# obeychoi0120/wseg

Hardware: AMD Instinct MI355X
Metric: training images/sec at B=16x448x448 (contrast_train step) (higher is better)
Workload: dtype bf16; 1 GPU; ResNet-38 contrast, synthetic VOC 448x448, B=16/GPU, procedural weights, dropout on, fused HIP loss; global_batch=16, parallelism=dp1, seed=0

## Files before the change

wseg_amd/csrc/conv_igemm.hip:

```cpp
#include <stdlib.h>
#include <algorithm>
#include "common.h"
#include "conv_wgrad_kernels.h"
#include "conv_probes.h"

namespace {

constexpr int BN = 128, ROWB = 128;
constexpr int B_TILE = BN * ROWB;
constexpr int EPI_LD = BN + 4;

struct Args {
  wseg_conv_desc d;
  int M;
  int taps;
  int cpt;
  int cpt2;
  int krow;
  int ntn;
  int nwg;
  int row0;
  int perm;
  int Q1, Q2;
};

struct PermRow { wseg_rowgeo g; int cls; long true_row; };
__device__ __forceinline__ PermRow perm_decode(const Args& a, int m) {
  const wseg_conv_desc& d = a.d;
  PermRow r;
  int rr = m, H = d.OH, W = d.OW, Q = a.Q1, seg = 0;
  if (d.OH2 != 0 && rr >= 4 * a.Q1) { rr -= 4 * a.Q1; H = d.OH2; W = d.OW2; Q = a.Q2; seg = 1; }
  const int cls = rr / Q, rem = rr - cls * Q;
  const int hw2 = (H >> 1) * (W >> 1), w2 = W >> 1;
  const int n = rem / hw2, rem2 = rem - n * hw2;
  const int i = rem2 / w2, j = rem2 - i * w2;
  r.g.oy = 2 * i + (cls >> 1); r.g.ox = 2 * j + (cls & 1);
  r.g.n_glob = seg ? d.N + n : n;
  r.g.IH = seg ? d.IH2 : d.IH; r.g.IW = seg ? d.IW2 : d.IW;
  r.g.in_base = seg ? (long)d.N * d.IH * d.IW + (long)n * d.IH2 * d.IW2 : (long)n * d.IH * d.IW;
  r.cls = seg * 4 + cls;
  r.true_row = seg ? (long)d.N * d.OH * d.OW + ((long)n * H + r.g.oy) * W + r.g.ox : ((long)n * H + r.g.oy) * W + r.g.ox;
  return r;
}

__device__ __forceinline__ float elu1(float x) { return x > 0.f ? x : expm1f(x); }

__device__ __forceinline__ void epilogue_coeffs(const wseg_conv_desc& d, int n0, int cv, float (&sc)[8], float (&sh)[8]) {
  const int oc_raw = n0 + cv;
  const int oc = oc_raw < d.OC ? oc_raw : 0;
#pragma unroll
  for (int e = 0; e < 8; ++e) { sc[e] = 1.f; sh[e] = 0.f; }
  if (d.scale != nullptr) load8<WSEG_F32>(d.scale, oc, sc);
  if (d.shift != nullptr) load8<WSEG_F32>(d.shift, oc, sh);
}

template <int DT, int EPI, int ROWS>
__device__ __forceinline__ void epilogue_image(const wseg_conv_desc& d, int M, const float* img, int m0, int n0, int tid,
                                               const float (&sc)[8], const float (&sh)[8]) {
  constexpr int NT = 256, GPR = BN / 8;
  constexpr int RPS = NT / GPR;
  constexpr int SWEEPS = ROWS / RPS;
  constexpr int CHK = SWEEPS < 4 ? SWEEPS : 4;
  static_assert(NT % GPR == 0 && ROWS % RPS == 0 && SWEEPS % CHK == 0, "epilogue geometry");
  const int cv = (tid % GPR) * 8;
  const int oc_raw = n0 + cv;
  const bool col_ok = oc_raw < d.OC;
  const int oc = col_ok ? oc_raw : 0;
  const bool has_pre = d.r_pre != nullptr, has_post = d.r_post != nullptr, has_mask = d.mask != nullptr;
  const bool has_drop = d.drop != nullptr;
#pragma unroll 1
  for (int c0 = 0; c0 < SWEEPS; c0 += CHK) {
    float rpre[CHK][8], rpost[CHK][8], mk[CHK][8], dr[CHK][8];
    size_t mrow[CHK];
    bool ok[CHK];
#pragma unroll
    for (int j = 0; j < CHK; ++j) {
      const int row = ((c0 + j) * NT + tid) / GPR;
      ok[j] = col_ok && (m0 + row) < M;
      mrow[j] = ok[j] ? (size_t)(m0 + row) : 0;
    }
    if (has_pre) {
#pragma unroll
      for (int j = 0; j < CHK; ++j) load8<DT>(d.r_pre, mrow[j] * d.ld_rpre + oc, rpre[j]);
    }
    if (has_post) {
#pragma unroll
      for (int j = 0; j < CHK; ++j) load8<DT>(d.r_post, mrow[j] * d.ld_rpost + oc, rpost[j]);
    }
    if (EPI == 1 && has_mask) {
#pragma unroll
      for (int j = 0; j < CHK; ++j) load8<DT>(d.mask, mrow[j] * d.ld_mask + oc, mk[j]);
    }
    if (EPI < 2 && has_drop) {
#pragma unroll
      for (int j = 0; j < CHK; ++j) load8<WSEG_F32>(d.drop, (size_t)wseg_decode_row(d, (int)mrow[j]).n_glob * d.OC + oc, dr[j]);
    }
#pragma unroll
    for (int j = 0; j < CHK; ++j) {
      const int row = ((c0 + j) * NT + tid) / GPR;
      const size_t m = mrow[j];
      float v[8];
      const f32x4 p0 = *reinterpret_cast<const f32x4*>(&img[row * EPI_LD + cv]);
      const f32x4 p1 = *reinterpret_cast<const f32x4*>(&img[row * EPI_LD + cv + 4]);
#pragma unroll
      for (int e = 0; e < 4; ++e) { v[e] = p0[e]; v[4 + e] = p1[e]; }
      if (has_pre) {
#pragma unroll
        for (int e = 0; e < 8; ++e) v[e] += rpre[j][e];
      }
      if constexpr (EPI == 0) {
        if (has_post) {
#pragma unroll
          for (int e = 0; e < 8; ++e) v[e] += rpost[j][e];
        }
        if (d.relu_lt > 0) {
#pragma unroll
          for (int e = 0; e < 8; ++e) if (oc + e < d.relu_lt) v[e] = fmaxf(v[e], 0.f);
        }
        if (d.out != nullptr && ok[j]) store8<DT>(d.out, m * d.ld_out + oc, v);
        if (d.out2 != nullptr) {
          float t[8];
#pragma unroll
          for (int e = 0; e < 8; ++e) {
            float x = v[e] * sc[e] + sh[e];
            if (d.relu_out2) x = fmaxf(x, 0.f);
            if (has_drop) x *= dr[j][e];
            t[e] = x;
          }
          if (ok[j]) store8<DT>(d.out2, m * d.ld_out2 + oc, t);
        }
      } else if constexpr (EPI == 1) {
        float o[8];
#pragma unroll
        for (int e = 0; e < 8; ++e) {
          float x = v[e] * sc[e];
          if (has_drop) x *= dr[j][e];
          if (has_mask) x = mk[j][e] > 0.f ? x : 0.f;
          if (has_post) x += rpost[j][e];
          o[e] = x;
        }
        if (ok[j]) store8<DT>(d.out, m * d.ld_out + oc, o);
      } else if constexpr (EPI == 2) {
#pragma unroll
        for (int e = 0; e < 8; ++e) v[e] = fmaxf(v[e], 0.f);
        if (ok[j]) store8<DT>(d.out, m * d.ld_out + oc, v);
      } else {
#pragma unroll
        for (int e = 0; e < 8; ++e) v[e] = elu1(v[e]);
        if (ok[j]) store8<DT>(d.out, m * d.ld_out + oc, v);
      }
    }
  }
}

template <int DT> struct raw8;
template <> struct raw8<WSEG_BF16> {
  uint4 q;
  __device__ __forceinline__ void load(const void* p, size_t i) { q = *reinterpret_cast<const uint4*>((const bf16_t*)p + i); }
  __device__ __forceinline__ void unpack(float (&v)[8]) const {
    const unsigned w[4] = {q.x, q.y, q.z, q.w};
#pragma unroll
    for (int j = 0; j < 4; ++j) { v[2 * j] = __uint_as_float(w[j] << 16); v[2 * j + 1] = __uint_as_float(w[j] & 0xFFFF0000u); }
  }
};
template <> struct raw8<WSEG_F32X3> {
  f32x4 q0, q1;
  __device__ __forceinline__ void load(const void* p, size_t i) {
    q0 = *reinterpret_cast<const f32x4*>((const float*)p + i); q1 = *reinterpret_cast<const f32x4*>((const float*)p + i + 4);
  }
  __device__ __forceinline__ void unpack(float (&v)[8]) const {
#pragma unroll
    for (int e = 0; e < 4; ++e) { v[e] = q0[e]; v[4 + e] = q1[e]; }
  }
};

template <int EPI, int NI, int I0, int NB, int DT>
__device__ __forceinline__ void wave_local_epilogue_batch(const Args& a, float* wimg, int lane, int mw0, int oc, bool col_ok,
                                                          const float (&sc)[8], const float (&sh)[8], const f32x4 (&acc)[NI][4]) {
  constexpr int WLD = 64 + 4;
  const wseg_conv_desc& d = a.d;
  const int frow = lane & 15, fk = lane >> 4;
  const int vr = lane >> 3, vg = lane & 7;
  const bool ld_ok_ = WSEG_DIAG_EPI_LOADS();
  const bool has_pre = d.r_pre != nullptr && ld_ok_, has_post = d.r_post != nullptr && ld_ok_, has_mask = EPI == 1 && d.mask != nullptr && ld_ok_;
  const bool has_drop = EPI < 2 && d.drop != nullptr && ld_ok_;
  const bool res_is_pre = has_pre;
  const bool post_in_step = has_pre && has_post;
  const void* res_p = res_is_pre ? d.r_pre : d.r_post;
  const size_t res_ld = res_is_pre ? d.ld_rpre : d.ld_rpost;
  const bool has_res = has_pre || has_post;
  int mrow[NB][2]; bool ok[NB][2];
  raw8<DT> qres[NB][2], qmk[NB][2];
#pragma unroll
  for (int i = 0; i < NB; ++i)
#pragma unroll
    for (int t = 0; t < 2; ++t) {
      const int m = mw0 + (I0 + i) * 16 + vr + 8 * t;
      ok[i][t] = col_ok && m < a.M;
      mrow[i][t] = ok[i][t] ? (a.perm ? (int)perm_decode(a, m).true_row : m) : 0;
      ok[i][t] = ok[i][t] && WSEG_DIAG_EPI_STORES();
      if (has_res) qres[i][t].load(res_p, (size_t)mrow[i][t] * res_ld + oc);
      if (has_mask) qmk[i][t].load(d.mask, (size_t)mrow[i][t] * d.ld_mask + oc);
    }
#pragma unroll
  for (int i = 0; i < NB; ++i) {
    float rpost[2][8], dr[2][8];
    if (post_in_step) {
#pragma unroll
      for (int t = 0; t < 2; ++t) load8<DT>(d.r_post, (size_t)mrow[i][t] * d.ld_rpost + oc, rpost[t]);
    }
    if (has_drop) {
#pragma unroll
      for (int t = 0; t < 2; ++t) load8<WSEG_F32>(d.drop, (size_t)wseg_decode_row(d, mrow[i][t]).n_glob * d.OC + oc, dr[t]);
    }
#pragma unroll
    for (int j = 0; j < 4; ++j)
#pragma unroll
      for (int e = 0; e < 4; ++e) wimg[(fk * 4 + e) * WLD + j * 16 + frow] = acc[I0 + i][j][e];
    asm volatile("s_waitcnt lgkmcnt(0)" ::: "memory");
#pragma unroll
    for (int t = 0; t < 2; ++t) {
      float v[8];
      {
        const f32x4 p0 = *reinterpret_cast<const f32x4*>(&wimg[(vr + 8 * t) * WLD + vg * 8]);
        const f32x4 p1 = *reinterpret_cast<const f32x4*>(&wimg[(vr + 8 * t) * WLD + vg * 8 + 4]);
#pragma unroll
        for (int e = 0; e < 4; ++e) { v[e] = p0[e]; v[4 + e] = p1[e]; }
      }
      const size_t m = (size_t)mrow[i][t];
      float res[8];
      if (has_res) qres[i][t].unpack(res);
      if (has_pre) {
#pragma unroll
        for (int e = 0; e < 8; ++e) v[e] += res[e];
      }
      if (!post_in_step && has_post) {
#pragma unroll
        for (int e = 0; e < 8; ++e) rpost[t][e] = res[e];
      }
      if constexpr (EPI == 0) {
        if (has_post) {
#pragma unroll
          for (int e = 0; e < 8; ++e) v[e] += rpost[t][e];
        }
        if (d.relu_lt > 0) {
#pragma unroll
          for (int e = 0; e < 8; ++e) if (oc + e < d.relu_lt) v[e] = fmaxf(v[e], 0.f);
        }
        if (d.out != nullptr && ok[i][t]) store8<DT>(d.out, m * d.ld_out + oc, v);
        if (d.out2 != nullptr) {
          float o2[8];
#pragma unroll
          for (int e = 0; e < 8; ++e) {
            float x = v[e] * sc[e] + sh[e];
            if (d.relu_out2) x = fmaxf(x, 0.f);
            if (has_drop) x *= dr[t][e];
            o2[e] = x;
          }
          if (ok[i][t]) store8<DT>(d.out2, m * d.ld_out2 + oc, o2);
        }
      } else if constexpr (EPI == 1) {
        float mk[8];
        if (has_mask) qmk[i][t].unpack(mk);
        float o[8];
#pragma unroll
        for (int e = 0; e < 8; ++e) {
          float x = v[e] * sc[e];
          if (has_drop) x *= dr[t][e];
          if (has_mask) x = mk[e] > 0.f ? x : 0.f;
          if (has_post) x += rpost[t][e];
          o[e] = x;
        }
        if (ok[i][t]) store8<DT>(d.out, m * d.ld_out + oc, o);
      } else if constexpr (EPI == 2) {
#pragma unroll
        for (int e = 0; e < 8; ++e) v[e] = fmaxf(v[e], 0.f);
        if (ok[i][t]) store8<DT>(d.out, m * d.ld_out + oc, v);
      } else {
#pragma unroll
        for (int e = 0; e < 8; ++e) v[e] = elu1(v[e]);
        if (ok[i][t]) store8<DT>(d.out, m * d.ld_out + oc, v);
      }
    }
    asm volatile("s_waitcnt lgkmcnt(0)" ::: "memory");
  }
}

template <int EPI, int NI, int DT, int I0, int NB>
__device__ __forceinline__ void wave_local_epilogue_rec(const Args& a, float* wimg, int lane, int mw0, int oc, bool col_ok,
                                                        const float (&sc)[8], const float (&sh)[8], const f32x4 (&acc)[NI][4]) {
  if constexpr (I0 < NI) {
    wave_local_epilogue_batch<EPI, NI, I0, (NI - I0 < NB ? NI - I0 : NB), DT>(a, wimg, lane, mw0, oc, col_ok, sc, sh, acc);
    wave_local_epilogue_rec<EPI, NI, DT, I0 + NB, NB>(a, wimg, lane, mw0, oc, col_ok, sc, sh, acc);
  }
}

template <int EPI, int NI, int DT = WSEG_BF16>
__device__ __forceinline__ void wave_local_epilogue(const Args& a, char* smem, int wid, int lane, int mw0, int col0, int n0,
                                                    const f32x4 (&acc)[NI][4]) {
  const wseg_conv_desc& d = a.d;
  constexpr int WLD = 64 + 4;
  float* wimg = reinterpret_cast<float*>(smem) + wid * (16 * WLD);
  const int vg = lane & 7;
  const int oc_raw = n0 + col0 + vg * 8;
  const bool col_ok = oc_raw < d.OC;
  const int oc = col_ok ? oc_raw : 0;
  float sc[8], sh[8];
  epilogue_coeffs(d, n0, col0 + vg * 8, sc, sh);
  constexpr int NB = DT == WSEG_BF16 ? 4 : 2;
  wave_local_epilogue_rec<EPI, NI, DT, 0, NB>(a, wimg, lane, mw0, oc, col_ok, sc, sh, acc);
}

template <int DT, int EPI, int BM>
__global__ __launch_bounds__(256, 2) void conv_igemm_kernel(const Args a) {
  constexpr int AI = BM / 32;
  constexpr int A_TILE = BM * ROWB;
  constexpr int STAGE = A_TILE + B_TILE;
  constexpr int SMEM_BYTES = (BM * EPI_LD * 4 > 2 * STAGE) ? BM * EPI_LD * 4 : 2 * STAGE;
  constexpr int ES = elem<DT>::size;
  constexpr int CH = 16 / ES;
  __shared__ __attribute__((aligned(16))) char smem[SMEM_BYTES];
  const wseg_conv_desc& d = a.d;

  const int tid = threadIdx.x, lane = tid & 63;
  const int wid = __builtin_amdgcn_readfirstlane(tid >> 6);
  const int tile = xcd_remap(blockIdx.x, a.nwg);
  const int tm = tile / a.ntn, tn = tile - tm * a.ntn;
  const int m0 = a.row0 + tm * BM, n0 = tn * BN;

  const char* zero = reinterpret_cast<const char*>(g_wseg_zero_page);
  const char* IN = reinterpret_cast<const char*>(d.in);
  const char* Wp = reinterpret_cast<const char*>(d.w);

  const int srow = lane >> 3;
  const int pch = lane & 7;
  int a_iy0[AI], a_ix0[AI], a_H[AI], a_W[AI];
  long a_img[AI];
  const char* bptr[4];
  int b_inc[4];
  int lch[4];
  int lcha[AI];
#pragma unroll
  for (int i = 0; i < AI; ++i) {
    const int r = wid * (BM / 4) + i * 8 + srow;
    lcha[i] = pch ^ ((r >> 1) & 7);
    const int m = m0 + r;
    if (m < a.M) {
      const wseg_rowgeo rg = wseg_decode_row(d, m);
      const int oy = rg.oy, ox = rg.ox;
      a_img[i] = rg.in_base; a_H[i] = rg.IH; a_W[i] = rg.IW;
      if (d.mode == 0) { a_iy0[i] = oy * d.stride - d.pad; a_ix0[i] = ox * d.stride - d.pad; }
      else             { a_iy0[i] = oy + d.pad;            a_ix0[i] = ox + d.pad; }
    } else {
      a_img[i] = -1; a_iy0[i] = 0; a_ix0[i] = 0; a_H[i] = 1; a_W[i] = 1;
    }
  }
#pragma unroll
  for (int i = 0; i < 4; ++i) {
    const int r = wid * 32 + i * 8 + srow;
    lch[i] = pch ^ ((r >> 1) & 7);
    const int oc = n0 + r;
    if (oc < d.OC) {
      bptr[i] = Wp + ((size_t)oc * a.taps * d.IC + (size_t)lch[i] * CH) * ES;
      b_inc[i] = ROWB;
    } else {
      bptr[i] = zero + pch * 16; b_inc[i] = 0;
    }
  }
  const char* aptr[AI];
  int a_inc[AI];
  auto set_tap = [&](int tap) {
    const int ky = tap / d.KW, kx = tap - ky * d.KW;
#pragma unroll
    for (int i = 0; i < AI; ++i) {
      int iy, ix; bool ok = a_img[i] >= 0;
      if (d.mode == 0) {
        iy = a_iy0[i] + ky * d.dil; ix = a_ix0[i] + kx * d.dil;
      } else {
        const int ty = a_iy0[i] - ky * d.dil, tx = a_ix0[i] - kx * d.dil;
        ok = ok && ty >= 0 && tx >= 0;
        if (d.stride == 1) { iy = ty; ix = tx; }
        else { iy = ty / d.stride; ix = tx / d.stride; ok = ok && (iy * d.stride == ty) && (ix * d.stride == tx); }
      }
      ok = ok && iy >= 0 && iy < a_H[i] && ix >= 0 && ix < a_W[i];
      if (ok) {
        aptr[i] = IN + ((size_t)(a_img[i] + (long)iy * a_W[i] + ix) * d.ld_in + (size_t)lcha[i] * CH) * ES;
        a_inc[i] = ROWB;
      } else {
        aptr[i] = zero + pch * 16; a_inc[i] = 0;
      }
    }
  };

  auto stage = [&](int buf) {
    char* la = smem + buf * STAGE + wid * (BM / 4) * ROWB;
    char* lb = smem + buf * STAGE + A_TILE + wid * 32 * ROWB;
#pragma unroll
    for (int i = 0; i < AI; ++i) {
      glds16(aptr[i], la + i * 8 * ROWB);
      aptr[i] += a_inc[i];
    }
#pragma unroll
    for (int i = 0; i < 4; ++i) {
      glds16(bptr[i], lb + i * 8 * ROWB);
      bptr[i] += b_inc[i];
    }
  };

  const int wr = wid >> 1, wc = wid & 1;
  const int frow = lane & 15, fk = lane >> 4;
  const int sw = (lane >> 1) & 7;
  const int a_rd = (wr * (BM / 2) + frow) * ROWB;
  const int b_rd = A_TILE + (wc * 64 + frow) * ROWB;

  f32x4 acc[AI][4];
#pragma unroll
  for (int i = 0; i < AI; ++i)
#pragma unroll
    for (int j = 0; j < 4; ++j) acc[i][j] = (f32x4){0.f, 0.f, 0.f, 0.f};

  const int nk = a.taps * a.cpt;
  int tap = 0, cc = 0;
  set_tap(0);
  stage(0);
  __syncthreads();
  int cur = 0;
  for (int kt = 0; kt < nk; ++kt) {
    if (kt + 1 < nk) {
      if (++cc == a.cpt) { cc = 0; ++tap; set_tap(tap); }
      stage(cur ^ 1);
    }
    const char* base = smem + cur * STAGE;
    if constexpr (DT == WSEG_F32X3) {
      bf16x8 ah[AI], al[AI], bh[4], bl[4];
#pragma unroll
      for (int i = 0; i < AI; ++i) {
        const f32x4 p0 = *reinterpret_cast<const f32x4*>(base + a_rd + i * 16 * ROWB + (((2 * fk) ^ sw) * 16));
        const f32x4 p1 = *reinterpret_cast<const f32x4*>(base + a_rd + i * 16 * ROWB + (((2 * fk + 1) ^ sw) * 16));
        split_bf16x8(p0, p1, ah[i], al[i]);
      }
#pragma unroll
      for (int j = 0; j < 4; ++j) {
        bh[j] = *reinterpret_cast<const bf16x8*>(base + b_rd + j * 16 * ROWB + ((fk ^ sw) * 16));
        bl[j] = *reinterpret_cast<const bf16x8*>(base + b_rd + j * 16 * ROWB + (((4 + fk) ^ sw) * 16));
      }
#pragma unroll
      for (int i = 0; i < AI; ++i)
#pragma unroll
        for (int j = 0; j < 4; ++j) {
          acc[i][j] = __builtin_amdgcn_mfma_f32_16x16x32_bf16(al[i], bh[j], acc[i][j], 0, 0, 0);
          acc[i][j] = __builtin_amdgcn_mfma_f32_16x16x32_bf16(ah[i], bl[j], acc[i][j], 0, 0, 0);
          acc[i][j] = __builtin_amdgcn_mfma_f32_16x16x32_bf16(ah[i], bh[j], acc[i][j], 0, 0, 0);
        }
    } else {
#pragma unroll
    for (int ks = 0; ks < 2; ++ks) {
      const int off = ((ks * 4 + fk) ^ sw) * 16;
      if constexpr (DT == WSEG_BF16) {
        bf16x8 af[AI], bf[4];
#pragma unroll
        for (int i = 0; i < AI; ++i) af[i] = *reinterpret_cast<const bf16x8*>(base + a_rd + i * 16 * ROWB + off);
#pragma unroll
        for (int i = 0; i < 4; ++i) bf[i] = *reinterpret_cast<const bf16x8*>(base + b_rd + i * 16 * ROWB + off);
#pragma unroll
        for (int i = 0; i < AI; ++i)
#pragma unroll
          for (int j = 0; j < 4; ++j)
            acc[i][j] = __builtin_amdgcn_mfma_f32_16x16x32_bf16(af[i], bf[j], acc[i][j], 0, 0, 0);
      } else {
        f32x4 af[AI], bf[4];
#pragma unroll
        for (int i = 0; i < AI; ++i) af[i] = *reinterpret_cast<const f32x4*>(base + a_rd + i * 16 * ROWB + off);
#pragma unroll
        for (int i = 0; i < 4; ++i) bf[i] = *reinterpret_cast<const f32x4*>(base + b_rd + i * 16 * ROWB + off);
#pragma unroll
        for (int e = 0; e < 4; ++e)
#pragma unroll
          for (int i = 0; i < AI; ++i)
#pragma unroll
            for (int j = 0; j < 4; ++j)
              acc[i][j] = __builtin_amdgcn_mfma_f32_16x16x4f32(af[i][e], bf[j][e], acc[i][j], 0, 0, 0);
      }
    }
    }
    __syncthreads();
    cur ^= 1;
  }

  float* img = reinterpret_cast<float*>(smem);
#pragma unroll
  for (int i = 0; i < AI; ++i)
#pragma unroll
    for (int j = 0; j < 4; ++j) {
      const int row = wr * (BM / 2) + i * 16 + fk * 4;
      const int col = wc * 64 + j * 16 + frow;
#pragma unroll
      for (int e = 0; e < 4; ++e) img[(row + e) * EPI_LD + col] = acc[i][j][e];
    }
  __syncthreads();

  float sc[8], sh[8];
  epilogue_coeffs(d, n0, (tid & 15) * 8, sc, sh);
  epilogue_image<DT, EPI, BM>(d, a.M, img, m0, n0, tid, sc, sh);
}

constexpr int HALF256 = 16384, TILE256 = 4 * HALF256;

template <int EPI, int NI = 8, int DT = WSEG_BF16, bool TAPF = true>
__device__ __forceinline__ void conv_igemm256_tile(const Args& a, char* smem, const int bid) {
  constexpr bool X3 = DT == WSEG_F32X3;
  constexpr int ES = X3 ? 4 : 2, CH = 16 / ES;
  constexpr int RH = NI * 16, BMT = 2 * RH;
  static_assert(NI == 8 || NI == 7, "256- or 224-row tiles");
  const wseg_conv_desc& d = a.d;
  const int tid = threadIdx.x, lane = tid & 63;
  const int wid = __builtin_amdgcn_readfirstlane(tid >> 6);
  const int tile = xcd_remap(bid, a.nwg);
  const int tm = tile / a.ntn, tn = tile - tm * a.ntn;
  const int m0 = a.row0 + tm * BMT, n0 = tn * 256;
  const int wr = wid >> 2, wc = wid & 3;
  const int frow = lane & 15, fk = lane >> 4, sw = (lane >> 1) & 7;
  WSEG_STAMP(0, 0);
  WSEG_DIAG_LOAD();

  const char* zero = reinterpret_cast<const char*>(g_wseg_zero_page);
  const char* IN = reinterpret_cast<const char*>(d.in);
  const char* Wp = reinterpret_cast<const char*>(d.w);

  const int r0 = tid >> 3, pch = tid & 7;
  const int lc = pch ^ ((r0 >> 1) & 7);
  const char* zsrc = zero + pch * 16;
  const char* INl = IN + lc * 16;
  unsigned long long tl = 0xFEDCBA9876543210ull;
  int ntaps = a.taps;
  if (a.perm) {
    const int c0 = perm_decode(a, m0).cls, c1 = perm_decode(a, min(m0 + BMT - 1, a.M - 1)).cls;
    if (c0 == c1) {
      const int py = (c0 >> 1) & 1, px = c0 & 1;
      tl = 0ull; ntaps = 0;
      for (int t = 0; t < a.taps; ++t) {
        const int ky = t / d.KW, kx = t - ky * d.KW;
        if ((((py + d.pad - ky * d.dil) | (px + d.pad - kx * d.dil)) & 1) == 0) { tl |= (unsigned long long)t << (4 * ntaps); ++ntaps; }
      }
      if (ntaps == 0) { tl = 0ull; ntaps = 1; }
    }
  }
  const char* bptr0 = Wp + ((size_t)(n0 + r0) * a.krow + (size_t)lc * CH) * ES;
  const char* bptr = bptr0 + (size_t)(tl & 15ull) * d.IC * ES;
  int b_ti = 0, b_cc = 0;
  const int brs = 64 * a.krow * ES;
  auto issue_b = [&](int h, int buf) {
    char* dst = smem + buf * TILE256 + (2 + h) * HALF256 + wid * 1024;
    glds16(bptr + (2 * h) * brs, dst);
    glds16(bptr + (2 * h + 1) * brs, dst + 8192);
  };
  auto advance_b = [&]() {
    bptr += 128;
    if (a.perm && ++b_cc == a.cpt) { b_cc = 0; ++b_ti; bptr = bptr0 + (size_t)((tl >> (4 * b_ti)) & 15ull) * d.IC * ES; }
  };

  const int nt = d.in2 != nullptr ? (ntaps - 1) * a.cpt + a.cpt2 : ntaps * a.cpt;
  issue_b(0, 0); issue_b(1, 0); advance_b();
  if (nt > 1) { issue_b(0, 1); issue_b(1, 1); advance_b(); }
  int a_w0[4], a_w1[4];
#pragma unroll
  for (int j = 0; j < 4; ++j) {
    const int rho = r0 + 64 * (j & 1);
    const int m = m0 + (j >> 1) * RH + rho;
    if constexpr (TAPF) {
      a_w0[j] = 0; a_w1[j] = 0;
      if (rho < RH && m < a.M) {
        const wseg_rowgeo rg = wseg_decode_row(d, m);
        const int sg = d.mode == 0 ? d.dil : -d.dil;
        const int iy0 = d.mode == 0 ? rg.oy * d.stride - d.pad : rg.oy + d.pad, ix0 = d.mode == 0 ? rg.ox * d.stride - d.pad : rg.ox + d.pad;
        unsigned mk = rg.n_glob >= d.N ? 0x10000u : 0u;
#pragma unroll
        for (int k = 0; k < 3; ++k) {
          if ((unsigned)(iy0 + k * sg) < (unsigned)rg.IH) mk |= 1u << k;
          if ((unsigned)(ix0 + k * sg) < (unsigned)rg.IW) mk |= 0x100u << k;
        }
        if (d.KH > 3 || d.KW > 3) {
          for (int k = 3; k < 8; ++k) {
            if ((unsigned)(iy0 + k * sg) < (unsigned)rg.IH) mk |= 1u << k;
            if ((unsigned)(ix0 + k * sg) < (unsigned)rg.IW) mk |= 0x100u << k;
          }
        }
        a_w0[j] = (int)rg.in_base + iy0 * rg.IW + ix0;
        a_w1[j] = (int)mk;
      }
    } else {
      if (rho < RH && m < a.M) {
        const wseg_rowgeo rg = a.perm ? perm_decode(a, m).g : wseg_decode_row(d, m);
        int iy0, ix0;
        if (d.mode == 0) { iy0 = rg.oy * d.stride - d.pad; ix0 = rg.ox * d.stride - d.pad; }
        else             { iy0 = rg.oy + d.pad;            ix0 = rg.ox + d.pad; }
        a_w0[j] = (int)rg.in_base;
        a_w1[j] = (rg.n_glob >= d.N ? (int)0x80000000 : 0) | ((iy0 + 0x2000) << 16) | (ix0 + 0x2000);
      } else {
        a_w0[j] = -1; a_w1[j] = (0x2000 << 16) | 0x2000;
      }
    }
  }
  const char* aptr[4];
  unsigned a_live = 0;
  int a_tap = 0, a_cc = 0;
  int a_ky = 0, a_kx = 0;
  auto set_tap = [&](int tap) {
    const bool src2 = d.in2 != nullptr && tap == d.KH * d.KW;
    const char* INs = src2 ? reinterpret_cast<const char*>(d.in2) + lc * 16 : INl;
    const int lds = src2 ? d.ld_in2 : d.ld_in;
    a_live = 0;
    if constexpr (TAPF) {
      const int tky = src2 ? d.KH / 2 : a_ky, tkx = src2 ? d.KW / 2 : a_kx;
      const int sg = d.mode == 0 ? d.dil : -d.dil;
      const int dp1 = sg * (tky * d.IW + tkx), dp2 = sg * (tky * d.IW2 + tkx);
      const unsigned tmask = (1u << tky) | (0x100u << tkx);
      const int rowb = lds * ES;
#pragma unroll
      for (int j = 0; j < 4; ++j) {
        const unsigned vm = (unsigned)a_w1[j];
        const bool ok = (vm & tmask) == tmask;
        const int off = (a_w0[j] + ((vm & 0x10000u) ? dp2 : dp1)) * rowb;
        const char* p = INs + (long)off;
        aptr[j] = ok ? p : zsrc;
        a_live |= ok ? 1u << j : 0u;
      }
    } else {
      const int tg = src2 ? (d.KH / 2) * d.KW + d.KW / 2 : tap;
      const int ky = tg / d.KW, kx = tg - ky * d.KW;
      const int (&a_base)[4] = a_w0; const int (&a_yx)[4] = a_w1;
#pragma unroll
    for (int j = 0; j < 4; ++j) {
      const int iy0 = ((a_yx[j] >> 16) & 0x7FFF) - 0x2000, ix0 = (a_yx[j] & 0xFFFF) - 0x2000;
      const bool s2 = a_yx[j] < 0;
      const int H = s2 ? d.IH2 : d.IH, W = s2 ? d.IW2 : d.IW;
      int iy, ix; bool ok = a_base[j] >= 0;
      if (d.mode == 0) {
        iy = iy0 + ky * d.dil; ix = ix0 + kx * d.dil;
      } else {
        const int ty = iy0 - ky * d.dil, tx = ix0 - kx * d.dil;
        ok = ok && ty >= 0 && tx >= 0;
        if (d.stride == 1) { iy = ty; ix = tx; }
        else { iy = ty / d.stride; ix = tx / d.stride; ok = ok && (iy * d.stride == ty) && (ix * d.stride == tx); }
      }
      ok = ok && iy >= 0 && iy < H && ix >= 0 && ix < W;
      if (ok) { aptr[j] = INs + (size_t)(a_base[j] + iy * W + ix) * lds * ES; a_live |= 1u << j; }
      else    { aptr[j] = zsrc; }
    }
    }
  };
  auto issue_a = [&](int h, int buf) {
    char* dst = smem + buf * TILE256 + h * HALF256 + wid * 1024;
    glds16(aptr[2 * h], dst);
    glds16(aptr[2 * h + 1], dst + 8192);
  };
  auto advance_a = [&]() {
#pragma unroll
    for (int j = 0; j < 4; ++j) aptr[j] += ((a_live >> j) & 1u) << 7;
    if (++a_cc == a.cpt) {
      a_cc = 0;
      if (++a_tap < ntaps) {
        if (TAPF) { if (++a_kx == d.KW) { a_kx = 0; ++a_ky; } }
        set_tap((int)((tl >> (4 * a_tap)) & 15ull));
      }
    }
  };
  f32x4 acc[NI][4];
#pragma unroll
  for (int i = 0; i < NI; ++i)
#pragma unroll
    for (int j = 0; j < 4; ++j) acc[i][j] = (f32x4){0.f, 0.f, 0.f, 0.f};

  set_tap((int)(tl & 15ull));
  issue_a(0, 0); issue_a(1, 0); advance_a();
  WSEG_STAMP(1, 0);
  asm volatile("s_waitcnt vmcnt(0)" ::: "memory");
  __builtin_amdgcn_s_barrier();
  WSEG_STAMP(2, 0);
#ifndef WSEG_SLOTS
  WSEG_CSTAMP(8, 0);
#endif

  bf16x8 af[2][4], b0[2][2], b1[2][2];
  auto ldA = [&](const char* aH, int ha) {
    if constexpr (X3) {
#pragma unroll
      for (int i = 0; i < 4; ++i)
        if (ha * 4 + i < NI) {
          const char* row = aH + (ha * 64 + i * 16 + frow) * 128;
          const f32x4 p0 = *reinterpret_cast<const f32x4*>(row + (((2 * fk) ^ sw) << 4));
          const f32x4 p1 = *reinterpret_cast<const f32x4*>(row + (((2 * fk + 1) ^ sw) << 4));
          split_bf16x8(p0, p1, af[0][i], af[1][i]);
        }
    } else {
#pragma unroll
    for (int ks = 0; ks < 2; ++ks)
#pragma unroll
      for (int i = 0; i < 4; ++i)
        if (ha * 4 + i < NI)
          af[ks][i] = *reinterpret_cast<const bf16x8*>(aH + (ha * 64 + i * 16 + frow) * 128 + (((ks * 4 + fk) ^ sw) << 4));
    }
  };
  auto ldB = [&](const char* bH, int hb, bf16x8 (&bf)[2][2]) {
#pragma unroll
    for (int ks = 0; ks < 2; ++ks)
#pragma unroll
      for (int j = 0; j < 2; ++j)
        bf[ks][j] = *reinterpret_cast<const bf16x8*>(bH + ((wc & 1) * 64 + hb * 32 + j * 16 + frow) * 128 + (((ks * 4 + fk) ^ sw) << 4));
  };
#define MFMA_Q(HA, HB, BF)                                                                                   \
  do {                                                                                                       \
    __builtin_amdgcn_s_setprio(1);                                                                           \
    if constexpr (X3) {                                                                                      \
      _Pragma("unroll") for (int i = 0; i < 4; ++i)                                                          \
        _Pragma("unroll") for (int j = 0; j < 2; ++j)                                                        \
          if ((HA) * 4 + i < NI) {                                                                           \
            f32x4& c_ = acc[(HA) * 4 + i][(HB) * 2 + j];                                                     \
            c_ = __builtin_amdgcn_mfma_f32_16x16x32_bf16(af[1][i], BF[0][j], c_, 0, 0, 0);                   \
            c_ = __builtin_amdgcn_mfma_f32_16x16x32_bf16(af[0][i], BF[1][j], c_, 0, 0, 0);                   \
            c_ = __builtin_amdgcn_mfma_f32_16x16x32_bf16(af[0][i], BF[0][j], c_, 0, 0, 0);                   \
          }                                                                                                  \
    } else                                                                                                   \
    _Pragma("unroll") for (int ks = 0; ks < 2; ++ks)                                                         \
      _Pragma("unroll") for (int i = 0; i < 4; ++i)                                                          \
        _Pragma("unroll") for (int j = 0; j < 2; ++j)                                                        \
          if ((HA) * 4 + i < NI)                              \
            acc[(HA) * 4 + i][(HB) * 2 + j] =                                                                \
                __builtin_amdgcn_mfma_f32_16x16x32_bf16(af[ks][i], BF[ks][j], acc[(HA) * 4 + i][(HB) * 2 + j], 0, 0, 0); \
    __builtin_amdgcn_s_setprio(0);                                                                           \
  } while (0)

  {
    WSEG_SLOT_DECL();
    if (wr == 1) __builtin_amdgcn_s_barrier();
    WSEG_SLOT_BEGIN();
    for (int u = 0; u < nt; ++u) {
      const int b = u & 1;
      const char* aH = smem + b * TILE256 + wr * HALF256;
      const char* bH = smem + b * TILE256 + (2 + (wc >> 1)) * HALF256;
      ldA(aH, 0); ldB(bH, 0, b0); ldB(bH, 1, b1);
      if (u + 1 < nt && WSEG_DIAG_A_OK(u)) { issue_a(0, b ^ 1); issue_a(1, b ^ 1); }
      WSEG_SLOT(0);
      __builtin_amdgcn_s_barrier();
      WSEG_SLOT(1);
      if (wr == 0 && u + 1 < nt && WSEG_DIAG_A_MOVES()) advance_a();
      MFMA_Q(0, 0, b0);
      MFMA_Q(0, 1, b1);
      WSEG_SLOT(2);
      __builtin_amdgcn_s_barrier();
      WSEG_SLOT(3);
      ldA(aH, 1);
      if (u + 2 < nt) { if (WSEG_DIAG_B_OK()) { issue_b(0, b); issue_b(1, b); } if (WSEG_DIAG_B_MOVES()) advance_b(); asm volatile("s_waitcnt vmcnt(4)" ::: "memory"); }
      else asm volatile("s_waitcnt vmcnt(0)" ::: "memory");
      WSEG_SLOT(4);
      __builtin_amdgcn_s_barrier();
      WSEG_SLOT(5);
      if (wr == 1 && u + 1 < nt && WSEG_DIAG_A_MOVES()) advance_a();
      MFMA_Q(1, 1, b1);
      MFMA_Q(1, 0, b0);
      WSEG_SLOT(6);
      __builtin_amdgcn_s_barrier();
      WSEG_SLOT(7);
    }
    WSEG_SLOT_FLUSH();
    if (wr == 0) __builtin_amdgcn_s_barrier();
  }
#undef MFMA_Q

  WSEG_STAMP(3, 0); WSEG_STAMP(5, 4);
#ifndef WSEG_SLOTS
  WSEG_CSTAMP(9, 0);
#endif
  __syncthreads();
  wave_local_epilogue<EPI, NI, DT>(a, smem, wid, lane, m0 + wr * RH, wc * 64, n0, acc);
#ifdef WSEG_PROBES
  asm volatile("s_waitcnt vmcnt(0)" ::: "memory");
  WSEG_STAMP(4, 0); WSEG_STAMP(6, 4);
  if (threadIdx.x == 0 && bid < 4096) g_wseg_stamps[bid * 24 + 7] = __builtin_amdgcn_s_getreg(20 | (0 << 6) | (3 << 11));
#endif
}

template <int EPI, int NI = 8, int DT = WSEG_BF16, bool TAPF = true>
__global__ __launch_bounds__(512, 2) void conv_igemm256_kernel(const Args a) {
  __shared__ __attribute__((aligned(16))) char smem[2 * TILE256];
  conv_igemm256_tile<EPI, NI, DT, TAPF>(a, smem, blockIdx.x);
}

constexpr int TILE5 = 5 * HALF256;

template <int EPI>
__global__ __launch_bounds__(512, 2) void conv_igemm512x128_kernel(const Args a) {
  constexpr int ES = 2, CH = 8;
  __shared__ __attribute__((aligned(16))) char smem[2 * TILE5];
  const wseg_conv_desc& d = a.d;
  const int tid = threadIdx.x, lane = tid & 63;
  const int wid = __builtin_amdgcn_readfirstlane(tid >> 6);
  const int tile = xcd_remap(blockIdx.x, a.nwg);
  const int tm = tile / a.ntn, tn = tile - tm * a.ntn;
  const int m0 = a.row0 + tm * 512, n0 = tn * 128;
  const int wr = wid >> 1, wc = wid & 1;
  const int frow = lane & 15, fk = lane >> 4, sw = (lane >> 1) & 7;

  const char* zero = reinterpret_cast<const char*>(g_wseg_zero_page);
  const char* IN = reinterpret_cast<const char*>(d.in);
  const char* Wp = reinterpret_cast<const char*>(d.w);

  const int r0 = tid >> 3, pch = tid & 7;
  const int lc = pch ^ ((r0 >> 1) & 7);
  const char* zsrc = zero + pch * 16;
  const char* INl = IN + lc * 16;
  const char* rowptr[8];
  int a_yx[8];
  unsigned segmask = 0;
#pragma unroll
  for (int j = 0; j < 8; ++j) {
    const int m = m0 + r0 + 64 * j;
    rowptr[j] = zsrc; a_yx[j] = 0;
    if (m < a.M) {
      const wseg_rowgeo rg = wseg_decode_row(d, m);
      int iy0, ix0;
      if (d.mode == 0) { iy0 = rg.oy * d.stride - d.pad; ix0 = rg.ox * d.stride - d.pad; }
      else             { iy0 = rg.oy + d.pad;            ix0 = rg.ox + d.pad; }
      a_yx[j] = ((iy0 + 0x2000) << 16) | (ix0 + 0x2000);
      segmask |= rg.n_glob >= d.N ? 1u << j : 0u;
      rowptr[j] = INl + ((long)rg.in_base + (long)iy0 * rg.IW + ix0) * d.ld_in * ES;
    }
  }
  unsigned a_ok = 0;
  long koff1 = 0, koff2 = 0;
  const char* bptr = Wp + ((size_t)(n0 + r0) * a.taps * d.IC + (size_t)lc * CH) * ES;
  const int brs = 64 * a.taps * d.IC * ES;
  int t_ky = 0, t_kx = 0;
  auto set_tap = [&]() {
    const int ky = t_ky, kx = t_kx;
    const int dyt = d.mode == 0 ? ky * d.dil : -ky * d.dil, dxt = d.mode == 0 ? kx * d.dil : -kx * d.dil;
    koff1 = ((long)dyt * d.IW + dxt) * d.ld_in * ES; koff2 = ((long)dyt * d.IW2 + dxt) * d.ld_in * ES;
    a_ok = 0;
#pragma unroll
    for (int j = 0; j < 8; ++j) {
      const bool s2 = (segmask >> j) & 1u;
      const unsigned H = s2 ? d.IH2 : d.IH, W = s2 ? d.IW2 : d.IW;
      const int iy = (a_yx[j] >> 16) - 0x2000 + dyt, ix = (a_yx[j] & 0xFFFF) - 0x2000 + dxt;
      a_ok |= ((unsigned)iy < H && (unsigned)ix < W) ? 1u << j : 0u;
    }
  };
  int a_tap = 0, a_cc = 0;
  auto issue_a = [&](int buf) {
#pragma unroll
    for (int j = 0; j < 8; ++j) {
      const char* p = rowptr[j] + (((segmask >> j) & 1u) ? koff2 : koff1);
      p = ((a_ok >> j) & 1u) ? p : zsrc;
      glds16(p, smem + buf * TILE5 + (j >> 1) * HALF256 + (j & 1) * 8192 + wid * 1024);
    }
  };
  auto advance_a = [&]() {
    koff1 += 128; koff2 += 128;
    if (++a_cc == a.cpt) {
      a_cc = 0;
      if (++a_tap < a.taps) { if (++t_kx == d.KW) { t_kx = 0; ++t_ky; } set_tap(); }
    }
  };
  auto issue_b = [&](int buf) {
    char* dst = smem + buf * TILE5 + 4 * HALF256 + wid * 1024;
    glds16(bptr, dst);
    glds16(bptr + brs, dst + 8192);
    bptr += 128;
  };

  f32x4 acc[8][4];
#pragma unroll
  for (int i = 0; i < 8; ++i)
#pragma unroll
    for (int j = 0; j < 4; ++j) acc[i][j] = (f32x4){0.f, 0.f, 0.f, 0.f};

  const int nt = a.taps * a.cpt;
  set_tap();
  issue_a(0); advance_a(); issue_b(0);
  if (nt > 1) { issue_b(1); asm volatile("s_waitcnt vmcnt(2)" ::: "memory"); }
  else asm volatile("s_waitcnt vmcnt(0)" ::: "memory");
  __builtin_amdgcn_s_barrier();

  bf16x8 af[2][4], bf[2][4];
  auto ldA = [&](const char* aH, int ha) {
#pragma unroll
    for (int ks = 0; ks < 2; ++ks)
#pragma unroll
      for (int i = 0; i < 4; ++i)
        af[ks][i] = *reinterpret_cast<const bf16x8*>(aH + (ha * 64 + i * 16 + frow) * 128 + (((ks * 4 + fk) ^ sw) << 4));
  };
#define MFMA_H5(HA)                                                                                          \
  do {                                                                                                       \
    __builtin_amdgcn_s_setprio(1);                                                                           \
    _Pragma("unroll") for (int ks = 0; ks < 2; ++ks)                                                         \
      _Pragma("unroll") for (int i = 0; i < 4; ++i)                                                          \
        _Pragma("unroll") for (int j = 0; j < 4; ++j)                                                        \
          acc[(HA) * 4 + i][j] = __builtin_amdgcn_mfma_f32_16x16x32_bf16(af[ks][i], bf[ks][j], acc[(HA) * 4 + i][j], 0, 0, 0); \
    __builtin_amdgcn_s_setprio(0);                                                                           \
  } while (0)

  const int grp = wr >> 1;
  if (grp == 1) __builtin_amdgcn_s_barrier();
  for (int u = 0; u < nt; ++u) {
    const int b = u & 1;
    const char* aH = smem + b * TILE5 + wr * HALF256;
    const char* bH = smem + b * TILE5 + 4 * HALF256;
    ldA(aH, 0);
#pragma unroll
    for (int ks = 0; ks < 2; ++ks)
#pragma unroll
      for (int j = 0; j < 4; ++j)
        bf[ks][j] = *reinterpret_cast<const bf16x8*>(bH + (wc * 64 + j * 16 + frow) * 128 + (((ks * 4 + fk) ^ sw) << 4));
    if (u + 1 < nt) issue_a(b ^ 1);
    __builtin_amdgcn_s_barrier();
    if (grp == 0 && u + 1 < nt) advance_a();
    MFMA_H5(0);
    __builtin_amdgcn_s_barrier();
    ldA(aH, 1);
    if (u + 2 < nt) { issue_b(b); asm volatile("s_waitcnt vmcnt(2)" ::: "memory"); }
    else asm volatile("s_waitcnt vmcnt(0)" ::: "memory");
    __builtin_amdgcn_s_barrier();
    if (grp == 1 && u + 1 < nt) advance_a();
    MFMA_H5(1);
    __builtin_amdgcn_s_barrier();
  }
  if (grp == 0) __builtin_amdgcn_s_barrier();
#undef MFMA_H5

  __syncthreads();
  wave_local_epilogue<EPI, 8>(a, smem, wid, lane, m0 + wr * 128, wc * 64, n0, acc);
}

template <int EPI, int NI, int UNIT>
__global__ __launch_bounds__(512, 2) void conv_bwd_pair_kernel(const Args ad, const wseg_wg::Args aw, const int nd_pad) {
  __shared__ __attribute__((aligned(16))) char smem[2 * TILE256];
  static_assert(2 * TILE256 == 2 * 4 * 16384, "both tile bodies use the same 128 KiB");
  const int b = blockIdx.x;
  if (b < nd_pad) {
    if (b < ad.nwg) conv_igemm256_tile<EPI, NI, WSEG_BF16>(ad, smem, b);
  } else {
    wseg_wg::conv_wgrad_pipe_tile<UNIT>(aw, smem, b - nd_pad);
  }
}

}

static bool conv_cost_prefers_256(long M, int OC) {
  const long t256 = ((M + 255) / 256) * ((OC + 255) / 256);
  const long rounds = (t256 + 255) / 256;
  const long t224 = ((M + 223) / 224) * ((OC + 255) / 256), t128 = ((M + 127) / 128) * ((OC + 127) / 128);
  const double c_big = std::min((double)rounds * 8.0, (double)((t224 + 255) / 256) * 7.0), c_128 = (double)((t128 + 511) / 512) * 5.33;
  return c_big <= c_128;
}
static bool conv_rounds_prefer_224(long M, int ntn256) {
  const long t8 = ((M + 255) / 256) * ntn256, t7 = ((M + 223) / 224) * ntn256;
  return ((t7 + 255) / 256) * 7 < ((t8 + 255) / 256) * 8;
}

struct ConvPlan { Args a; int family; bool tapf; };

static int conv_plan(const wseg_conv_desc* d, ConvPlan& p) {
  WSEG_CHECK(d && d->in && d->w && (d->out || d->out2), "conv_igemm: null pointer");
  WSEG_CHECK(d->dtype == WSEG_F32 || d->dtype == WSEG_BF16 || d->dtype == WSEG_F32X3, "conv_igemm: bad dtype %d", d->dtype);
  const int es = d->dtype == WSEG_BF16 ? 2 : 4;
  WSEG_CHECK((d->IC * es) % ROWB == 0, "conv_igemm: IC=%d must be a multiple of %d", d->IC, ROWB / es);
  WSEG_CHECK(d->OC % 8 == 0 && d->ld_in % 8 == 0, "conv_igemm: OC=%d / ld_in=%d must be multiples of 8", d->OC, d->ld_in);
  WSEG_CHECK(d->N > 0 && d->OH > 0 && d->OW > 0 && d->IH > 0 && d->IW > 0, "conv_igemm: empty shape");
  WSEG_CHECK(d->stride >= 1 && d->dil >= 1 && d->KH >= 1 && d->KW >= 1, "conv_igemm: bad geometry");
  WSEG_CHECK(d->mode == 0 || d->mode == 1, "conv_igemm: bad mode");
  WSEG_CHECK(d->epi >= 0 && d->epi <= 3, "conv_igemm: bad epilogue");
  WSEG_CHECK(d->ld_in >= d->IC, "conv_igemm: ld_in < IC");
  if (d->out) WSEG_CHECK(d->ld_out >= d->OC && d->ld_out % 8 == 0, "conv_igemm: bad ld_out");
  if (d->out2) WSEG_CHECK(d->ld_out2 >= d->OC && d->ld_out2 % 8 == 0 && d->epi == 0, "conv_igemm: bad out2");
  if (d->r_pre) WSEG_CHECK(d->ld_rpre % 8 == 0, "conv_igemm: bad ld_rpre");
  if (d->r_post) WSEG_CHECK(d->ld_rpost % 8 == 0, "conv_igemm: bad ld_rpost");
  if (d->mask) WSEG_CHECK(d->ld_mask % 8 == 0, "conv_igemm: bad ld_mask");
  const long M = (long)d->N * d->OH * d->OW + (long)d->N * d->OH2 * d->OW2;
  const long in_rows = (long)d->N * d->IH * d->IW + (long)d->N * d->IH2 * d->IW2;
  WSEG_CHECK(d->OH2 >= 0 && (d->OH2 == 0 || (d->OW2 > 0 && d->IH2 > 0 && d->IW2 > 0)), "conv_igemm: bad second segment");
  WSEG_CHECK(d->w_rows == 0 || d->w_rows >= d->OC, "conv_igemm: w_rows=%d < OC=%d", d->w_rows, d->OC);
  WSEG_CHECK(M < (1L << 31) && (long)d->N * d->IH * d->IW * d->ld_in < (1L << 40), "conv_igemm: tensor too large");
  if (d->in2)
    WSEG_CHECK(d->KH == d->KW && (d->KH & 1) && d->KH * d->KW < 15 && d->stride == 1 && d->pad == d->dil * (d->KH / 2) &&
               d->dtype == WSEG_BF16 && d->OC % 256 == 0 && d->ld_in2 % 8 == 0 && d->epi != 3 && (d->bm_hint == 0 || d->bm_hint == 256 || d->bm_hint == 224),
               "conv_igemm: the two-source form is a same-size stride-1 bf16 convolution with OC %% 256 == 0 on the 256-tile kernel");
  const int ic2 = d->in2 ? (d->IC2 > 0 ? d->IC2 : d->IC) : 0;
  WSEG_CHECK(!d->in2 || ((ic2 * es) % ROWB == 0 && d->ld_in2 >= ic2), "conv_igemm: IC2=%d must be a multiple of %d and <= ld_in2", ic2, ROWB / es);
  WSEG_CHECK(d->out || d->epi == 0, "conv_igemm: epilogue %d needs `out`", d->epi);
  WSEG_CHECK(d->bm_hint != 257 && d->bm_hint != 258 && d->bm_hint >= 0, "conv_igemm: bm_hint %d was a development hook and no longer exists", d->bm_hint);

  Args& a = p.a;
  a.d = *d;
  a.perm = 0; a.Q1 = a.Q2 = 0;
  a.M = (int)M;
  a.row0 = 0;
  a.taps = d->KH * d->KW + (d->in2 ? 1 : 0);
  a.cpt = d->IC * es / ROWB;
  a.cpt2 = ic2 * es / ROWB;
  a.krow = d->KH * d->KW * d->IC + ic2;
  p.tapf = false;

  const bool oc_ok = d->OC % 256 == 0 || (d->in2 == nullptr && d->w_rows >= ((d->OC + 255) / 256) * 256);
  const bool can256 = (d->dtype == WSEG_BF16 || d->dtype == WSEG_F32X3) && oc_ok && d->epi != 3 && d->bm_hint != 64 && d->bm_hint != 128 &&
                      d->bm_hint != 259 && d->KH <= 8 && d->KW <= 8 && a.taps <= 16;
  if (can256 && (d->bm_hint == 256 || d->bm_hint == 224 || d->in2 != nullptr || conv_cost_prefers_256(M, d->OC))) {
    WSEG_CHECK(d->IH <= 16384 && d->IW <= 16384 && d->OH <= 16384 && d->OW <= 16384 && d->pad <= 4096 && in_rows < (1L << 31),
               "conv_igemm: shape too large for the 256-tile kernel");
    if (d->mode == 1 && d->stride == 2 && d->OH % 2 == 0 && d->OW % 2 == 0 && d->OH2 % 2 == 0 && d->OW2 % 2 == 0 && a.taps <= 9 &&
        (a.taps > 1 || d->bm_hint == 256)) {
      a.perm = 1;
      a.Q1 = d->N * (d->OH / 2) * (d->OW / 2);
      a.Q2 = d->N * (d->OH2 / 2) * (d->OW2 / 2);
    }
    a.ntn = (d->OC + 255) / 256;
    const bool ni7 = d->bm_hint == 224 || (d->bm_hint == 0 && conv_rounds_prefer_224(M, a.ntn));
    p.family = ni7 ? WSEG_CONV_224x256 : WSEG_CONV_256x256;
    a.nwg = (int)(((M + (ni7 ? 223 : 255)) / (ni7 ? 224 : 256)) * a.ntn);
    p.tapf = !(d->mode == 1 && d->stride != 1) && in_rows * std::max(d->ld_in, d->in2 ? d->ld_in2 : 0) * es < (1L << 31) - (1L << 24);
    return 0;
  }
  if (d->dtype == WSEG_BF16 && d->epi != 3 && d->OC % 128 == 0 && (d->mode == 0 || d->stride == 1) &&
      (d->bm_hint == 259 || (d->bm_hint == 0 && d->OC == 128 && (M + 511) / 512 >= 512))) {
    WSEG_CHECK(d->IH <= 8000 && d->IW <= 8000 && d->OH <= 8000 && d->OW <= 8000 && d->pad <= 4096 && d->KH * d->dil <= 4096,
               "conv_igemm: shape too large for the 512x128-tile kernel");
    p.family = WSEG_CONV_512x128;
    a.ntn = d->OC / 128;
    a.nwg = (int)(((M + 511) / 512) * a.ntn);
    return 0;
  }
  a.ntn = (d->OC + BN - 1) / BN;
  const bool small = d->bm_hint == 64 || (d->bm_hint != 128 && ((M + 127) / 128) * a.ntn < 384 && M > 64);
  p.family = small ? WSEG_CONV_64x128 : WSEG_CONV_128x128;
  a.nwg = (int)(((M + (small ? 63 : 127)) / (small ? 64 : 128)) * a.ntn);
  return 0;
}

static void conv_plan_report(const ConvPlan& p, wseg_launch_plan* out) {
  static const int rows[] = {0, 64, 128, 224, 256, 512};
  const bool t256 = p.family == WSEG_CONV_224x256 || p.family == WSEG_CONV_256x256;
  *out = wseg_launch_plan{p.family, rows[p.family], t256 ? 256 : 128, p.a.nwg, p.a.perm, p.tapf, 0, 0};
}

static void conv_launch(const ConvPlan& p, hipStream_t s) {
  const Args& a = p.a;
  const dim3 grid(a.nwg);
  switch (p.family) {
    case WSEG_CONV_224x256:
    case WSEG_CONV_256x256:
      with_const<3>(a.d.epi, [&](auto epi) {
        with_const<2>(p.family == WSEG_CONV_256x256, [&](auto ni8) {
          with_const<2>(a.d.dtype == WSEG_F32X3, [&](auto x3) {
            with_const<2>(p.tapf, [&](auto tapf) {
              constexpr int DT = decltype(x3)::value ? WSEG_F32X3 : WSEG_BF16;
              hipLaunchKernelGGL((conv_igemm256_kernel<decltype(epi)::value, 7 + decltype(ni8)::value, DT, decltype(tapf)::value != 0>), grid, dim3(512), 0, s, a);
            });
          });
        });
      });
      break;
    case WSEG_CONV_512x128:
      with_const<3>(a.d.epi, [&](auto epi) { hipLaunchKernelGGL(conv_igemm512x128_kernel<decltype(epi)::value>, grid, dim3(512), 0, s, a); });
      break;
    default:
      with_const<3>(a.d.dtype, [&](auto dt) {
        with_const<4>(a.d.epi, [&](auto epi) {
          with_const<2>(p.family == WSEG_CONV_128x128, [&](auto tall) {
            hipLaunchKernelGGL((conv_igemm_kernel<decltype(dt)::value, decltype(epi)::value, decltype(tall)::value ? 128 : 64>), grid, dim3(256), 0, s, a);
          });
        });
      });
  }
}

extern "C" int wseg_conv_plan(const wseg_conv_desc* d, wseg_launch_plan* out) {
  ConvPlan p;
  WSEG_CHECK(out, "conv_plan: null output");
  if (int rc = conv_plan(d, p)) return rc;
  conv_plan_report(p, out);
  return 0;
}

extern "C" int wseg_conv_igemm(const wseg_conv_desc* d, void* stream) {
  ConvPlan p;
  if (int rc = conv_plan(d, p)) return rc;
  conv_launch(p, (hipStream_t)stream);
  WSEG_LAUNCH_CHECK();
  return 0;
}

static int conv_bwd_pair_plan(const wseg_conv_desc* dg, const wseg_wgrad_desc* wg, ConvPlan& cp, wseg_wg::Plan& wp) {
  WSEG_CHECK(dg && wg, "conv_bwd_pair: null descriptor");
  if (int rc = conv_plan(dg, cp)) return rc;
  if (int rc = wseg_wg::wgrad_plan(wg, wp)) return rc;
  static const int pair_ok = getenv("WSEG_BWD_PAIR") ? atoi(getenv("WSEG_BWD_PAIR")) : 1;
  return pair_ok && (cp.family == WSEG_CONV_224x256 || cp.family == WSEG_CONV_256x256) && cp.tapf && !cp.a.perm && dg->dtype == WSEG_BF16 &&
         dg->mode == 1 && dg->bm_hint == 0 && dg->out2 == nullptr && wp.pipe;
}

extern "C" int wseg_conv_bwd_pair_plan(const wseg_conv_desc* dg, const wseg_wgrad_desc* wg, wseg_launch_plan* dg_plan, wseg_launch_plan* wg_plan) {
  ConvPlan cp; wseg_wg::Plan wp;
  WSEG_CHECK(dg_plan && wg_plan, "conv_bwd_pair_plan: null output");
  const int fuse = conv_bwd_pair_plan(dg, wg, cp, wp);
  if (fuse < 0) return fuse;
  conv_plan_report(cp, dg_plan);
  wseg_wg::wgrad_plan_report(wp, wg_plan);
  return fuse;
}

extern "C" int wseg_conv_bwd_pair(const wseg_conv_desc* dg, const wseg_wgrad_desc* wg, void* stream) {
  ConvPlan cp; wseg_wg::Plan wp;
  const int fuse = conv_bwd_pair_plan(dg, wg, cp, wp);
  if (fuse < 0) return fuse;
  hipStream_t s = (hipStream_t)stream;
  if (!fuse) {
    conv_launch(cp, s);
    WSEG_LAUNCH_CHECK();
    return wseg_conv_wgrad(wg, stream);
  }
  const Args& a = cp.a;
  const int nd_pad = (a.nwg + 7) & ~7;
  const dim3 grid((unsigned)(nd_pad + wp.a.nwg));
  with_const<3>(dg->epi, [&](auto epi) {
    with_const<2>(cp.family == WSEG_CONV_256x256, [&](auto ni8) {
      with_const<2>(wp.unit, [&](auto unit) {
        hipLaunchKernelGGL((conv_bwd_pair_kernel<decltype(epi)::value, 7 + decltype(ni8)::value, decltype(unit)::value>), grid, dim3(512), 0, s, a, wp.a, nd_pad);
      });
    });
  });
  WSEG_LAUNCH_CHECK();
  return 0;
}
```

Measured before the change: 472.8 images/sec.

## Pipeline epilogue residual/mask loads as a rolling prefetch ring and cache dropout rows

Replaces the batched epilogue, which issued all residual and mask loads for a group of accumulator rows and then drained them, with a rolling ring. The next row step's loads are issued right after the current step is consumed. Residual and mask presence become compile-time template parameters, with a smaller ring when both are present, to limit register pressure. Dropout factors are now loaded once and reloaded only when the decoded sample index changes, removing redundant per-row dropout loads. The reload path adds a full vmcnt wait and more template instantiations, which may grow code size and registers.

```diff
diff --git a/wseg_amd/csrc/conv_igemm.hip b/wseg_amd/csrc/conv_igemm.hip
--- a/wseg_amd/csrc/conv_igemm.hip
+++ b/wseg_amd/csrc/conv_igemm.hip
@@ -174,49 +174,56 @@
   }
 };
 
-template <int EPI, int NI, int I0, int NB, int DT>
-__device__ __forceinline__ void wave_local_epilogue_batch(const Args& a, float* wimg, int lane, int mw0, int oc, bool col_ok,
+template <int EPI, int NI, int DT, bool RES, bool MASK>
+__device__ __forceinline__ void wave_local_epilogue_steps(const Args& a, float* wimg, int lane, int mw0, int oc, bool col_ok,
                                                           const float (&sc)[8], const float (&sh)[8], const f32x4 (&acc)[NI][4]) {
+  constexpr int NB = (RES && MASK) ? (DT == WSEG_BF16 ? (NI == 7 ? 4 : 3) : 1) : (DT == WSEG_BF16 ? 4 : 2);
   constexpr int WLD = 64 + 4;
   const wseg_conv_desc& d = a.d;
   const int frow = lane & 15, fk = lane >> 4;
   const int vr = lane >> 3, vg = lane & 7;
   const bool ld_ok_ = WSEG_DIAG_EPI_LOADS();
-  const bool has_pre = d.r_pre != nullptr && ld_ok_, has_post = d.r_post != nullptr && ld_ok_, has_mask = EPI == 1 && d.mask != nullptr && ld_ok_;
+  constexpr bool has_res = RES, has_mask = MASK;
+  const bool has_pre = RES && d.r_pre != nullptr, has_post = RES && d.r_post != nullptr;
   const bool has_drop = EPI < 2 && d.drop != nullptr && ld_ok_;
   const bool res_is_pre = has_pre;
   const bool post_in_step = has_pre && has_post;
   const void* res_p = res_is_pre ? d.r_pre : d.r_post;
   const size_t res_ld = res_is_pre ? d.ld_rpre : d.ld_rpost;
-  const bool has_res = has_pre || has_post;
   int mrow[NB][2]; bool ok[NB][2];
   raw8<DT> qres[NB][2], qmk[NB][2];
-#pragma unroll
-  for (int i = 0; i < NB; ++i)
+  auto request = [&](int step, int s) {
 #pragma unroll
     for (int t = 0; t < 2; ++t) {
-      const int m = mw0 + (I0 + i) * 16 + vr + 8 * t;
-      ok[i][t] = col_ok && m < a.M;
-      mrow[i][t] = ok[i][t] ? (a.perm ? (int)perm_decode(a, m).true_row : m) : 0;
-      ok[i][t] = ok[i][t] && WSEG_DIAG_EPI_STORES();
-      if (has_res) qres[i][t].load(res_p, (size_t)mrow[i][t] * res_ld + oc);
-      if (has_mask) qmk[i][t].load(d.mask, (size_t)mrow[i][t] * d.ld_mask + oc);
-    }
-#pragma unroll
-  for (int i = 0; i < NB; ++i) {
-    float rpost[2][8], dr[2][8];
+      const int m = mw0 + step * 16 + vr + 8 * t;
+      ok[s][t] = col_ok && m < a.M;
+      mrow[s][t] = ok[s][t] ? (a.perm ? (int)perm_decode(a, m).true_row : m) : 0;
+      ok[s][t] = ok[s][t] && WSEG_DIAG_EPI_STORES();
+      if (has_res) qres[s][t].load(res_p, (size_t)mrow[s][t] * res_ld + oc);
+      if (has_mask) qmk[s][t].load(d.mask, (size_t)mrow[s][t] * d.ld_mask + oc);
+    }
+  };
+  float dr[8];
+  int dr_n = -1;
+  if (has_drop) {
+    const int m = mw0 + vr;
+    dr_n = wseg_decode_row(d, (col_ok && m < a.M) ? (a.perm ? (int)perm_decode(a, m).true_row : m) : 0).n_glob;
+    load8<WSEG_F32>(d.drop, (size_t)dr_n * d.OC + oc, dr);
+  }
+#pragma unroll
+  for (int i = 0; i < (NB < NI ? NB : NI); ++i) request(i, i);
+#pragma unroll
+  for (int i = 0; i < NI; ++i) {
+    const int s = i % NB;
+    float rpost[2][8];
     if (post_in_step) {
 #pragma unroll
-      for (int t = 0; t < 2; ++t) load8<DT>(d.r_post, (size_t)mrow[i][t] * d.ld_rpost + oc, rpost[t]);
-    }
-    if (has_drop) {
-#pragma unroll
-      for (int t = 0; t < 2; ++t) load8<WSEG_F32>(d.drop, (size_t)wseg_decode_row(d, mrow[i][t]).n_glob * d.OC + oc, dr[t]);
+      for (int t = 0; t < 2; ++t) load8<DT>(d.r_post, (size_t)mrow[s][t] * d.ld_rpost + oc, rpost[t]);
     }
 #pragma unroll
     for (int j = 0; j < 4; ++j)
 #pragma unroll
-      for (int e = 0; e < 4; ++e) wimg[(fk * 4 + e) * WLD + j * 16 + frow] = acc[I0 + i][j][e];
+      for (int e = 0; e < 4; ++e) wimg[(fk * 4 + e) * WLD + j * 16 + frow] = acc[i][j][e];
     asm volatile("s_waitcnt lgkmcnt(0)" ::: "memory");
 #pragma unroll
     for (int t = 0; t < 2; ++t) {
@@ -227,9 +234,17 @@
 #pragma unroll
         for (int e = 0; e < 4; ++e) { v[e] = p0[e]; v[4 + e] = p1[e]; }
       }
-      const size_t m = (size_t)mrow[i][t];
+      const size_t m = (size_t)mrow[s][t];
+      if (has_drop) {
+        const int n = wseg_decode_row(d, mrow[s][t]).n_glob;
+        if (n != dr_n) {
+          load8<WSEG_F32>(d.drop, (size_t)n * d.OC + oc, dr);
+          __builtin_amdgcn_s_waitcnt(0x0F70);
+          dr_n = n;
+        }
+      }
       float res[8];
-      if (has_res) qres[i][t].unpack(res);
+      if (has_res) qres[s][t].unpack(res);
       if (has_pre) {
 #pragma unroll
         for (int e = 0; e < 8; ++e) v[e] += res[e];
@@ -247,51 +262,43 @@
 #pragma unroll
           for (int e = 0; e < 8; ++e) if (oc + e < d.relu_lt) v[e] = fmaxf(v[e], 0.f);
         }
-        if (d.out != nullptr && ok[i][t]) store8<DT>(d.out, m * d.ld_out + oc, v);
+        if (d.out != nullptr && ok[s][t]) store8<DT>(d.out, m * d.ld_out + oc, v);
         if (d.out2 != nullptr) {
           float o2[8];
 #pragma unroll
           for (int e = 0; e < 8; ++e) {
             float x = v[e] * sc[e] + sh[e];
             if (d.relu_out2) x = fmaxf(x, 0.f);
-            if (has_drop) x *= dr[t][e];
+            if (has_drop) x *= dr[e];
             o2[e] = x;
           }
-          if (ok[i][t]) store8<DT>(d.out2, m * d.ld_out2 + oc, o2);
+          if (ok[s][t]) store8<DT>(d.out2, m * d.ld_out2 + oc, o2);
         }
       } else if constexpr (EPI == 1) {
         float mk[8];
-        if (has_mask) qmk[i][t].unpack(mk);
+        if (has_mask) qmk[s][t].unpack(mk);
         float o[8];
 #pragma unroll
         for (int e = 0; e < 8; ++e) {
           float x = v[e] * sc[e];
-          if (has_drop) x *= dr[t][e];
+          if (has_drop) x *= dr[e];
           if (has_mask) x = mk[e] > 0.f ? x : 0.f;
           if (has_post) x += rpost[t][e];
           o[e] = x;
         }
-        if (ok[i][t]) store8<DT>(d.out, m * d.ld_out + oc, o);
+        if (ok[s][t]) store8<DT>(d.out, m * d.ld_out + oc, o);
       } else if constexpr (EPI == 2) {
 #pragma unroll
         for (int e = 0; e < 8; ++e) v[e] = fmaxf(v[e], 0.f);
-        if (ok[i][t]) store8<DT>(d.out, m * d.ld_out + oc, v);
+        if (ok[s][t]) store8<DT>(d.out, m * d.ld_out + oc, v);
       } else {
 #pragma unroll
         for (int e = 0; e < 8; ++e) v[e] = elu1(v[e]);
-        if (ok[i][t]) store8<DT>(d.out, m * d.ld_out + oc, v);
-      }
-    }
+        if (ok[s][t]) store8<DT>(d.out, m * d.ld_out + oc, v);
+      }
+    }
+    if (i + NB < NI) request(i + NB, s);
     asm volatile("s_waitcnt lgkmcnt(0)" ::: "memory");
-  }
-}
-
-template <int EPI, int NI, int DT, int I0, int NB>
-__device__ __forceinline__ void wave_local_epilogue_rec(const Args& a, float* wimg, int lane, int mw0, int oc, bool col_ok,
-                                                        const float (&sc)[8], const float (&sh)[8], const f32x4 (&acc)[NI][4]) {
-  if constexpr (I0 < NI) {
-    wave_local_epilogue_batch<EPI, NI, I0, (NI - I0 < NB ? NI - I0 : NB), DT>(a, wimg, lane, mw0, oc, col_ok, sc, sh, acc);
-    wave_local_epilogue_rec<EPI, NI, DT, I0 + NB, NB>(a, wimg, lane, mw0, oc, col_ok, sc, sh, acc);
   }
 }
 
@@ -307,8 +314,17 @@
   const int oc = col_ok ? oc_raw : 0;
   float sc[8], sh[8];
   epilogue_coeffs(d, n0, col0 + vg * 8, sc, sh);
-  constexpr int NB = DT == WSEG_BF16 ? 4 : 2;
-  wave_local_epilogue_rec<EPI, NI, DT, 0, NB>(a, wimg, lane, mw0, oc, col_ok, sc, sh, acc);
+  const bool ld_ok_ = WSEG_DIAG_EPI_LOADS();
+  const bool has_res = (d.r_pre != nullptr || d.r_post != nullptr) && ld_ok_, has_mask = EPI == 1 && d.mask != nullptr && ld_ok_;
+  if constexpr (EPI == 1) {
+    if (has_mask) {
+      if (has_res) wave_local_epilogue_steps<EPI, NI, DT, true, true>(a, wimg, lane, mw0, oc, col_ok, sc, sh, acc);
+      else wave_local_epilogue_steps<EPI, NI, DT, false, true>(a, wimg, lane, mw0, oc, col_ok, sc, sh, acc);
+      return;
+    }
+  }
+  if (has_res) wave_local_epilogue_steps<EPI, NI, DT, true, false>(a, wimg, lane, mw0, oc, col_ok, sc, sh, acc);
+  else wave_local_epilogue_steps<EPI, NI, DT, false, false>(a, wimg, lane, mw0, oc, col_ok, sc, sh, acc);
 }
 
 template <int DT, int EPI, int BM>
```

Result: no change. 474.1 images/sec, median of 2 (+0.3%).
